# AberHu/TF-NAS

Hardware: AMD Instinct MI355X
Metric: supernet search images/sec (w-step + alpha-step) (higher is better)
Workload: dtype fp32

## Files before the change

tf-nas_amd/csrc/dw_stream.inc:

```

__device__ __forceinline__ int ring_swz(int c) { return c ^ ((c >> 2) & 1); }
struct WinBase {
    const float* b[2][2];
    __device__ __forceinline__ void set(const float* rowp, int d0, int d1) {
        b[0][0] = rowp + d0; b[0][1] = rowp - d0; b[1][0] = rowp + d1; b[1][1] = rowp - d1;
    }
    __device__ __forceinline__ const float* at(int u) const { return b[(u >> 2) & 1][u & 1]; }
};

__device__ __forceinline__ void dws_decode(const DwSlide& gm, int& cy, int& lane) {
    const int L = blockIdx.x;
    if (gm.gx & 7) {
        cy = L % gm.chunks;
        lane = L / gm.chunks;
    } else {
        const int x = L & 7, q = L >> 3;
        cy = q % gm.chunks;
        lane = (q / gm.chunks) * 8 + x;
    }
}

typedef unsigned u32x4 __attribute__((ext_vector_type(4)));
#ifndef TFNAS_LD_AUX
#define TFNAS_LD_AUX 2
// ... 226 lines not shown
                    slot = (slot + 1 == RB) ? 0 : slot + 1;
                }
            } else {
#pragma unroll 1
                for (int ky = 0; ky < K; ++ky) {
                    const float* rowp = ring_item + slot * ge.row_floats;
                    WinBase wb;
                    wb.set(rowp, swz0, swz1);
                    const float* wp = wts_item + ky * K * CC;
                    f32x4 win[K + 3];
#pragma unroll
                    for (int u = 0; u < K + 3; ++u) win[u] = ld4(wb.at(u) + u * CCP);
#pragma unroll
                    for (int kx = 0; kx < K; ++kx) {
                        const f32x4 wv = ld4(wp + kx * CC);
#pragma unroll
                        for (int j = 0; j < 4; ++j) acc[j] += win[j + kx] * wv;
                    }
                    slot = (slot + 1 == RB) ? 0 : slot + 1;
                }
            }
            const unsigned o = ge.row_off(ii, hh) + ooff;
#pragma unroll
            for (int j = 0; j < 4; ++j) {
                if (j < npx) {
                    bD.st4(o + (unsigned)(j * M), acc[j]);
                    ssum += acc[j];
                    ssq += acc[j] * acc[j];
                }
            }
        }
        spos.advance(TH, H, PAD, RB);
        __syncthreads();
        if (PIPE) {
            if (more) {
                rb.commit(ring, ge, bpos, xf);
                bpos.advance(TH, H, PAD, RB);
            }
            __syncthreads();
        }
    }
    dw_flush_stats(ssum, ssq, ring, CC, c0, mcp, off, M, part, lane);
}

template <int K, int ACT, bool PIPE, int KQ = 0, bool WGR = false>
__global__ __launch_bounds__(256, WGR ? 2 : ((PIPE || KQ > 0) ? 3 : 4)) void k_dws_bwd(TfnasCellDesc d, const float* __restrict__ dZ,
                                                    const float* __restrict__ gate, const float* __restrict__ dpooled,
                                                    const float* __restrict__ D, const double* __restrict__ stats2,
                                                    const double* __restrict__ red2, const float* __restrict__ E,
                                                    const double* __restrict__ stats1, float* __restrict__ dEh,
                                                    float* __restrict__ part, DwSlide gm,
                                                    const float* __restrict__ x = nullptr,
                                                    float* __restrict__ wpart = nullptr, size_t wout_size = 0) {
    static_assert(!(PIPE && KQ > 0), "the E-free variant has no register-prefetch form");
    static_assert(!(WGR && KQ > 0), "the fused weight gradient needs a materialised E");
    extern __shared__ __attribute__((aligned(16))) float lds[];
    int cy, lane, g, c0;
    dws_decode(gm, cy, lane);
    if (!dw_locate<K>(d, cy, gm.CC, g, c0)) return;
    const int mc = d.g[g].mc, mcp = d.g[g].mcp, off = d.g[g].off;
    constexpr int CC = 32, CCP = 32, CQ = CC >> 2;
    const int TH = gm.TH, L1 = gm.L1, RB = gm.RB;
    const int H = d.H, W = d.W, M = d.M;
    constexpr int PAD = K / 2;
    const int tid = threadIdx.x;

    float* ring = lds;
    float* wts = lds + RB * L1 * CCP;
    f32x4* cst2 = reinterpret_cast<f32x4*>(wts + K * K * CC);
    float2* cst1 = reinterpret_cast<float2*>(cst2 + CC);
    float* eht = reinterpret_cast<float*>(cst1 + CC);
    fill_cst2(cst2, d, CC, c0, mc, off, stats2, red2);
    if (tid < CC)
        cst1[tid] = (c0 + tid < mc) ? bn_consts(stats1 + 2 * (size_t)(off + c0 + tid), 1.0 / ((double)d.N * H * W), d.eps)
                                    : make_float2(0.f, 0.f);
    for (int idx = tid; idx < K * K * CC; idx += 256) {
        const int cl = idx % CC, t = idx / CC;
        wts[t * CC + cl] = (c0 + cl < mc) ? d.g[g].w_dw[(size_t)(c0 + cl) * (K * K) + (K * K - 1 - t)] : 0.f;
    }
    __syncthreads();
    ExpandB<(KQ > 0 ? KQ : 2)> xb;
    if (KQ > 0) expand_b_load(xb, d.g[g].w_expand, d.ic, c0, mc, cst1);

    StreamGeo ge;
    ge.H = H; ge.PAD = PAD; ge.RB = RB; ge.TH = TH;
    ge.nimg = (d.N - lane + gm.gx - 1) / gm.gx;
    ge.WM = (unsigned)W * M;
    ge.img_stride = (unsigned)gm.gx * H * ge.WM;
    ge.lane_base = (unsigned)lane * H * ge.WM + off + c0;
    ge.row_floats = L1 * CCP;
    const int nsteps = (ge.nimg * (H + PAD) + PAD + TH - 1) / TH;

    const int cq = tid & (CQ - 1);
    const bool has_se = d.g[g].se > 0;
    const float inv_hw = 1.f / (float)(H * W);
    f32x4 c2r[4];
    float2 c1r[4];
#pragma unroll
    for (int j = 0; j < 4; ++j) {
        c2r[j] = cst2[4 * cq + j];
        c1r[j] = cst1[4 * cq + j];
    }
    const float* gate_c = gate + off + c0 + 4 * cq;
    const float* dpool_c = dpooled + off + c0 + 4 * cq;
    auto xf = [&](f32x4 dz, f32x4 dv, int i) {
        f32x4 g4 = zero4(), dp4 = zero4();
        if (has_se) {
            const size_t n = (size_t)(lane + i * gm.gx) * M;
            g4 = ld4(gate_c + n);
            dp4 = ld4(dpool_c + n) * splat4(inv_hw);
        }
        return bn2_dd<ACT>(c2r, 0, dz, dv, has_se, g4, dp4);
    };
    const size_t numel = (size_t)d.N * H * W * M;
    BufView bZ, bDd, bE, bO;
    bZ.bind(dZ, numel);
    bDd.bind(D, numel);
    bE.bind(E, numel);
    bO.bind(dEh, numel);
    RingBlock<true> rb;
    rb.init(gm, W, M, mcp - c0, PAD);
    StreamPos bpos = {0, -PAD, 0};
    if (PIPE) {
        rb.issue(ge, bpos, bZ, bDd);
        rb.commit(ring, ge, bpos, xf);
        bpos.advance(TH, H, PAD, RB);
        __syncthreads();
    }

    const int nsw = gm.TW >> 2, st = tid >> gm.cq_shift;
    const int oh = st / nsw, ow0 = (st - oh * nsw) * 4;
    const bool item_ok = oh < TH && c0 + 4 * cq < mcp;
    const int npx = W - ow0 < 4 ? W - ow0 : 4;
    const float* ring_item = ring + ow0 * CCP + 4 * cq;
    const int swz0 = ((ow0 >> 2) & 1) * CCP, swz1 = CCP - swz0;
    const float* wts_item = wts + 4 * cq;
    const unsigned ooff = (unsigned)(ow0 * M + 4 * cq);
    StreamPos spos = {-1, H - PAD, RB - 2 * PAD};

    f32x4 t1 = zero4(), t2 = zero4();
    f32x4 wacc[WGR ? K * K : 1];
#pragma unroll
    for (int u = 0; u < (WGR ? K * K : 1); ++u) wacc[u] = zero4();
    for (int s = 0; s < nsteps; ++s) {
        const bool more = s + 1 < nsteps;
        if (PIPE) {
            if (more) rb.issue(ge, bpos, bZ, bDd);
        } else {
            rb.issue(ge, bpos, bZ, bDd);
            if (KQ > 0) {
                const int TW = gm.TW;
                const float inv_tw = 1.f / (float)TW;
                expand_tile_to<(KQ > 0 ? KQ : 2), 2>(
                    TH * TW, x, xb,
                    [&](int p, size_t& a) {
                        const int r = (int)(((float)p + 0.5f) * inv_tw), col = p - r * TW;
                        int bi, bh;
                        ge.locate(spos, r, bi, bh);
                        a = (((size_t)(lane + bi * gm.gx) * H + bh) * W + col) * d.ic;
                        return col < W && bh >= 0 && bi >= 0 && bi < ge.nimg;
                    },
                    [&](int p) { return eht + p * CCP; });
            }
            rb.commit(ring, ge, bpos, xf);
            bpos.advance(TH, H, PAD, RB);
            __syncthreads();
        }
        int ii, hh;
        ge.locate(spos, oh, ii, hh);
        if (item_ok && hh >= 0 && ii >= 0 && ii < ge.nimg) {
            const unsigned o = ge.row_off(ii, hh) + ooff;
            f32x4 ev[4];
#pragma unroll
            for (int j = 0; j < 4; ++j) {
                if (KQ > 0) ev[j] = ld4(eht + (oh * gm.TW + ow0 + j) * CCP + 4 * cq);
                else ev[j] = bE.ld4(j < npx ? o + (unsigned)(j * M) : BUF_OOB);
            }
            int slot = ge.slot_of(spos, oh);
            f32x4 acc[4] = {zero4(), zero4(), zero4(), zero4()};
            if (!WGR) {
#pragma unroll 1
                for (int ky = 0; ky < K; ++ky) {
                    const float* rowp = ring_item + slot * ge.row_floats;
                    WinBase wb;
                    wb.set(rowp, swz0, swz1);
                    const float* wp = wts_item + ky * K * CC;
                    f32x4 win[K + 3];
#pragma unroll
                    for (int u = 0; u < K + 3; ++u) win[u] = ld4(wb.at(u) + u * CCP);
#pragma unroll
                    for (int kx = 0; kx < K; ++kx) {
                        const f32x4 wv = ld4(wp + kx * CC);
#pragma unroll
                        for (int j = 0; j < 4; ++j) acc[j] += win[j + kx] * wv;
                    }
                    slot = (slot + 1 == RB) ? 0 : slot + 1;
                }
            } else {
                f32x4 a1v[4];
#pragma unroll
                for (int j = 0; j < 4; ++j)
#pragma unroll
                    for (int q = 0; q < 4; ++q)
                        a1v[j][q] = j < npx ? act_f<ACT>((ev[j][q] - c1r[q].x) * c1r[q].y) : 0.f;
#pragma unroll
                for (int ky = 0; ky < K; ++ky) {
                    const float* rowp = ring_item + slot * ge.row_floats;
                    WinBase wb;
                    wb.set(rowp, swz0, swz1);
                    const float* wp = wts_item + ky * K * CC;
                    f32x4 win[K + 3];
#pragma unroll
                    for (int u = 0; u < K + 3; ++u) win[u] = ld4(wb.at(u) + u * CCP);
#pragma unroll
                    for (int kx = 0; kx < K; ++kx) {
                        const f32x4 wv = ld4(wp + kx * CC);
#pragma unroll
                        for (int j = 0; j < 4; ++j) {
                            acc[j] += win[j + kx] * wv;
                            wacc[(K - 1 - ky) * K + (K - 1 - kx)] += a1v[j] * win[j + kx];
                        }
                    }
                    slot = (slot + 1 == RB) ? 0 : slot + 1;
                    __builtin_amdgcn_sched_barrier(0);
                }
            }
#pragma unroll
            for (int j = 0; j < 4; ++j) {
                if (j < npx) {
                    f32x4 deh;
#pragma unroll
                    for (int q = 0; q < 4; ++q) {
                        const float eh = KQ > 0 ? ev[j][q] : (ev[j][q] - c1r[q].x) * c1r[q].y;
                        deh[q] = acc[j][q] * act_d<ACT>(eh);
                        t1[q] += deh[q];
                        t2[q] += deh[q] * eh;
                    }
                    bO.st4(o + (unsigned)(j * M), deh);
                }
            }
        }
        spos.advance(TH, H, PAD, RB);
        __syncthreads();
        if (PIPE) {
            if (more) {
                rb.commit(ring, ge, bpos, xf);
                bpos.advance(TH, H, PAD, RB);
            }
            __syncthreads();
        }
    }
    dw_flush_stats(t1, t2, ring, CC, c0, mcp, off, M, part, lane);
    if (WGR) {
        for (int o = CQ; o < 64; o <<= 1) {
#pragma unroll
            for (int u = 0; u < K * K; ++u) {
#pragma unroll
                for (int q = 0; q < 4; ++q) wacc[u][q] += __shfl_xor(wacc[u][q], o, 64);
            }
        }
        __syncthreads();
        float* wred = ring;
        const int wl = tid & 63, wv = tid >> 6;
        if (wl < CQ) {
#pragma unroll
            for (int u = 0; u < K * K; ++u) st4(wred + (wv * K * K + u) * CC + 4 * wl, wacc[u]);
        }
        __syncthreads();
        size_t poff = 0;
        for (int gg = 0; gg < g; ++gg) poff += (size_t)d.g[gg].mc * d.g[gg].k * d.g[gg].k;
        float* __restrict__ gw = wpart + (size_t)lane * wout_size + poff;
        for (int idx = tid; idx < K * K * CC; idx += 256) {
            const int cl = idx % CC, u = idx / CC;
            if (c0 + cl < mc) {
                float sum = 0.f;
#pragma unroll
                for (int ww = 0; ww < 4; ++ww) sum += wred[(ww * K * K + u) * CC + cl];
                gw[(size_t)(c0 + cl) * (K * K) + u] = sum;
            }
        }
    }
}

template <int K, int ACT, bool PIPE>
__global__ __launch_bounds__(256, (!PIPE && K == 3) ? 4 : 2) void k_dws_wgrad(TfnasCellDesc d, const float* __restrict__ dZ,
                                                      const float* __restrict__ gate, const float* __restrict__ dpooled,
// ... 161 lines not shown
```

tf-nas_amd/csrc/dwconv_kernels.hip:

```cpp
#include <cstring>
#include <type_traits>
#include "tfnas_dev.h"
#include "kernels.h"
#include "prof.h"
#include "efree.h"

__device__ __forceinline__ int floordiv(int a, int b) { return a >= 0 ? a / b : -((-a + b - 1) / b); }

__device__ __forceinline__ int xcd_first_tile() {
    const int gx = gridDim.x, bx = blockIdx.x;
    return (gx & 7) ? bx : (bx & 7) * (gx >> 3) + (bx >> 3);
}

template <int K>
__device__ __forceinline__ bool dw_locate(const TfnasCellDesc& d, int cy, int CC, int& g, int& c0) {
    for (g = 0; g < d.G; ++g) {
        if (d.g[g].k != K) continue;
        const int t = (d.g[g].mcp + CC - 1) / CC;
        if (cy < t) {
            c0 = cy * CC;
            return true;
        }
        cy -= t;
    }
// ... 664 lines not shown
        else occ = dwd_bwd_occ(kk, d.stride, jw);
        const int want = 1024 * occ * wscale / 100;
        int ns = want / (gms[i].chunks * ncg);
        if (ns > steps / minper) ns = steps / minper;
        ns &= ~3;
        if (ns < 4) ns = 4;
        if (ns < nseg) nseg = ns;
    }
    size_t cap = TFNAS_PART_FLOATS / (row_floats ? row_floats : 1);
    if (cap > 1024) cap = 1024;
    while (nseg > 4 && (size_t)ncg * (nseg >> 2) > cap) nseg -= 4;
    if ((size_t)ncg * (nseg >> 2) > cap) return false;
    for (int i = 0; i < 2; ++i) {
        gms[i].ncg = ncg;
        gms[i].nseg = nseg;
        gms[i].steps = steps_k[i];
        gms[i].per = cdiv(steps_k[i], nseg);
        gms[i].nwg = gms[i].chunks * ncg * (nseg >> 2);
        p.chunks[i] = gms[i].chunks;
    }
    p.fam = DW_DIRECT;
    p.rows = ncg * (nseg >> 2);
    p.jw = jw;
    return true;
}

static DwPlan dw_plan_fwd(const TfnasCellDesc& d, bool efree, bool has_x) {
    DwPlan p = {};
    const size_t row = 2 * (size_t)d.M;
    if (!efree && dwd_fwd_use(d) && dwd_plan(d, row, dwd_jw(d), 1, p)) return p;
    p.kq = efree ? d.ic / 4 : 0;
    if ((!efree || (dws_efree_ic(d.ic) && has_x)) && dws_plan(d, row, p)) {
        p.pipe = !efree && dws_pipe(d);
        return p;
    }
    dw_tile_plan(d, d.Ho, d.Wo, true, 4096, row, efree, p);
    return p;
}

DwPlan dw_plan_bwd_data(const TfnasCellDesc& d, bool efree, bool has_x) {
    DwPlan p = {};
    const size_t row = 2 * (size_t)d.M, wout = dw_wout_size(d);
    const bool direct = !efree && dwd_bwd_use(d);
    if (direct) {
        const int jw = d.stride == 2 ? 2 : dwd_jw(d);
        p.fuse_wgrad = d.need_wgrad && !(d.route & TFNAS_ROUTE_DWWG2_OFF) && d.stride == 2 && dw_groups_k(d, true) &&
                       dwd_plan(d, row + wout + 64, jw, 2, p);
        if (p.fuse_wgrad || dwd_plan(d, row, jw, 2, p)) return p;
    }
    p.kq = efree ? d.ic / 4 : 0;
    if ((!efree || (dws_efree_ic(d.ic) && has_x)) && dws_plan(d, row, p)) {
        p.fuse_wgrad = !direct && !efree && d.need_wgrad && !(d.route & TFNAS_ROUTE_DWWG_OFF) && dw_groups_k(d, false) &&
                       d.W >= 28 && (size_t)p.rows * (row + 64 + wout) <= TFNAS_PART_FLOATS;
        p.pipe = !efree && !p.fuse_wgrad && dws_pipe(d);
        return p;
    }
    dw_tile_plan(d, d.H, d.W, false, 4096, row, efree, p);
    return p;
}

static DwPlan dw_plan_wgrad(const TfnasCellDesc& d) {
    DwPlan p = {};
    const size_t wout = dw_wout_size(d);
    if (dwd_wgrad_use(d) && dwd_plan(d, wout, dwd_jw(d), 0, p)) return p;
    if (dws_plan(d, wout, p)) {
        p.pipe = dws_pipe(d);
        return p;
    }
    dw_tile_plan(d, d.Ho, d.Wo, true, 2048, wout, false, p);
    return p;
}

template <int... Vs, class F>
static bool dw_dispatch(int k, int stride, int act, int v, F&& f) {
    bool hit = false;
    auto with_v = [&](auto K, auto S, auto A) {
        ((v == Vs ? (f(K, S, A, std::integral_constant<int, Vs>{}), hit = true) : false) || ...);
    };
    auto with_a = [&](auto K, auto S) {
        if (act == TFNAS_ACT_RELU) with_v(K, S, std::integral_constant<int, 0>{});
        else with_v(K, S, std::integral_constant<int, 1>{});
    };
    auto with_s = [&](auto K) {
        if (stride == 1) with_a(K, std::integral_constant<int, 1>{});
        else with_a(K, std::integral_constant<int, 2>{});
    };
    if (k == 3) with_s(std::integral_constant<int, 3>{});
    else with_s(std::integral_constant<int, 5>{});
    return hit;
}
constexpr int DW_WG = -1;
static int dws_variant(const DwPlan& p) { return p.fuse_wgrad ? DW_WG : p.kq ? p.kq : (int)p.pipe; }

static int dw_reduce_wgrad(const TfnasCellDesc& d, const float* wpart, int rows, size_t wout, hipStream_t s) {
    size_t poff = 0;
    for (int g = 0; g < d.G; ++g) {
        const int n = d.g[g].mc * d.g[g].k * d.g[g].k;
        const int rc = launch_reduce_rows(wpart + poff, rows, n, wout, nullptr, d.g[g].g_dw, s, wgrad_accum(d));
        if (rc) return rc;
        poff += n;
    }
    return 0;
}

int launch_dw_fwd(const TfnasCellDesc& d, const float* E, const float* x, const double* stats1, float* D,
                  double* stats2, float* part, hipStream_t s) {
    if (!E && !efree_ic_ok(d.ic)) return TFNAS_EINVAL;
    const DwPlan p = dw_plan_fwd(d, E == nullptr, x != nullptr);
    for (int i = 0; i < 2; ++i) {
        if (!p.chunks[i]) continue;
        const int kk = 3 + 2 * i;
        ProfScope _prof(TK_DW_FWD, s, d.G > 2);
        bool ok = false;
        if (p.fam == DW_DIRECT) {
            const DwDirect gm = p.direct[i];
            ok = dw_dispatch<2, 4>(kk, d.stride, d.act, p.jw, [&](auto K, auto S, auto A, auto JW) {
                hipLaunchKernelGGL((k_dwd_fwd<K, S, A, JW>), dim3(gm.nwg), dim3(256), 0, s, d, E, stats1, D, part, gm);
            });
        } else if (p.fam == DW_RING) {
            const DwSlide gm = p.ring[i];
            const size_t shm = (size_t)(gm.RB * gm.L1 * gm.CCP + kk * kk * gm.CC + 2 * gm.CC) * sizeof(float);
            ok = dw_dispatch<0, 1, 6, 10>(kk, d.stride, d.act, dws_variant(p), [&](auto K, auto, auto A, auto V) {
                hipLaunchKernelGGL((k_dws_fwd<K, A, V == 1, V == 1 ? 0 : V>), dim3(p.rows * gm.chunks), dim3(256), shm, s, d, E,
                                   stats1, D, part, gm, V > 1 ? x : nullptr);
            });
        } else {
            const DwGeom gm = p.tile[i];
            const int tile = gm.L0 * gm.L1 * gm.CC > 2048 ? gm.L0 * gm.L1 * gm.CC : 2048;
            const size_t shm = (size_t)(tile + kk * kk * gm.CC + 2 * gm.CC) * sizeof(float);
            if (shm > 64 * 1024) return TFNAS_ERANGE;
            ok = dw_dispatch<0, 4, 6, 10>(kk, d.stride, d.act, p.kq, [&](auto K, auto S, auto A, auto KQ) {
                hipLaunchKernelGGL((k_dw_fwd<K, S, A, KQ>), dim3(p.rows, p.chunks[i]), dim3(256), shm, s, d, E, x, stats1, D,
                                   part, gm);
            });
        }
        if (!ok) return TFNAS_EINVAL;
    }
    return launch_reduce_rows(part, p.rows, 2 * d.M, 2 * (size_t)d.M, stats2, nullptr, s);
}

int launch_dw_bwd_data(const DwPlan& p, const TfnasCellDesc& d, const float* dZ, const float* gate, const float* dpooled,
                       const float* D, const double* stats2, const double* red2, const float* E, const float* x,
                       const double* stats1, float* dEh, double* red1, float* part, hipStream_t s, float* cb1) {
    if (!E && !efree_ic_ok(d.ic)) return TFNAS_EINVAL;
    const size_t wout = dw_wout_size(d);
    float* wpart = part + (((size_t)p.rows * 2 * d.M + 63) & ~(size_t)63);
    for (int i = 0; i < 2; ++i) {
        if (!p.chunks[i]) continue;
        const int kk = 3 + 2 * i;
        ProfScope _prof(TK_DW_BWD_DATA, s, d.G > 2);
        bool ok = false;
        if (p.fam == DW_DIRECT) {
            const DwDirect gm = p.direct[i];
            ok = dw_dispatch<2, 4, DW_WG>(kk, d.stride, d.act, p.fuse_wgrad ? DW_WG : p.jw, [&](auto K, auto S, auto A, auto V) {
                if constexpr (V == DW_WG)
                    hipLaunchKernelGGL((k_dwd_bwd<K, 2, A, 2, true>), dim3(gm.nwg), dim3(256), 0, s, d, dZ, gate, dpooled, D,
                                       stats2, red2, E, stats1, dEh, part, gm, wpart, wout);
                else
                    hipLaunchKernelGGL((k_dwd_bwd<K, S, A, V>), dim3(gm.nwg), dim3(256), 0, s, d, dZ, gate, dpooled, D, stats2,
                                       red2, E, stats1, dEh, part, gm);
            });
        } else if (p.fam == DW_RING) {
            const DwSlide gm = p.ring[i];
            size_t shm = (size_t)(gm.RB * gm.L1 * gm.CCP + kk * kk * gm.CC + 4 * gm.CC + 2 * gm.CC +
                                  (p.kq ? gm.TH * gm.TW * gm.CCP : 0)) * sizeof(float);
            if (p.fuse_wgrad && shm < (size_t)4 * kk * kk * gm.CC * sizeof(float)) shm = (size_t)4 * kk * kk * gm.CC * sizeof(float);
            ok = dw_dispatch<0, 1, 6, 10, DW_WG>(kk, d.stride, d.act, dws_variant(p), [&](auto K, auto, auto A, auto V) {
                if constexpr (V == DW_WG) {
                    if constexpr (K == 3)
                        hipLaunchKernelGGL((k_dws_bwd<K, A, false, 0, true>), dim3(p.rows * gm.chunks), dim3(256), shm, s, d, dZ,
                                           gate, dpooled, D, stats2, red2, E, stats1, dEh, part, gm, nullptr, wpart, wout);
                } else {
                    hipLaunchKernelGGL((k_dws_bwd<K, A, V == 1, V == 1 ? 0 : V>), dim3(p.rows * gm.chunks), dim3(256), shm, s, d,
                                       dZ, gate, dpooled, D, stats2, red2, E, stats1, dEh, part, gm, V > 1 ? x : nullptr);
                }
            });
        } else {
            const DwGeom gm = p.tile[i];
            const int tile = gm.L0 * gm.L1 * gm.CC > 2048 ? gm.L0 * gm.L1 * gm.CC : 2048;
            const size_t shm = (size_t)(tile + kk * kk * gm.CC + 4 * gm.CC + 2 * gm.CC + (p.kq ? gm.T0 * gm.T1 * gm.CC : 0)) *
                               sizeof(float);
            if (shm > 64 * 1024) return TFNAS_ERANGE;
            ok = dw_dispatch<0, 4, 6, 10>(kk, d.stride, d.act, p.kq, [&](auto K, auto S, auto A, auto KQ) {
                hipLaunchKernelGGL((k_dw_bwd_data<K, S, A, KQ>), dim3(p.rows, p.chunks[i]), dim3(256), shm, s, d, dZ, gate,
                                   dpooled, D, stats2, red2, E, x, stats1, dEh, part, gm);
            });
        }
        if (!ok) return TFNAS_EINVAL;
    }
    if (p.fuse_wgrad) {
        ProfScope _prof(TK_DW_WGRAD, s);
        const int rc = dw_reduce_wgrad(d, wpart, p.rows, wout, s);
        if (rc) return rc;
    }
    if (cb1) return launch_reduce_bn1(d, part, p.rows, stats1, red1, cb1, s);
    return launch_reduce_rows(part, p.rows, 2 * d.M, 2 * (size_t)d.M, red1, nullptr, s);
}

int launch_dw_wgrad(const TfnasCellDesc& d, const float* dZ, const float* gate, const float* dpooled, const float* D,
                    const double* stats2, const double* red2, const float* E, const double* stats1, float* part,
                    hipStream_t s) {
    const DwPlan p = dw_plan_wgrad(d);
    const size_t wout = dw_wout_size(d);
    for (int i = 0; i < 2; ++i) {
        if (!p.chunks[i]) continue;
        const int kk = 3 + 2 * i;
        ProfScope _prof(TK_DW_WGRAD, s);
        if (p.fam == DW_DIRECT) {
            const DwDirect gm = p.direct[i];
            dw_dispatch<2, 4>(kk, d.stride, d.act, p.jw, [&](auto K, auto S, auto A, auto JW) {
                hipLaunchKernelGGL((k_dwd_wgrad<K, S, A, JW>), dim3(gm.nwg), dim3(256), 0, s, d, dZ, gate, dpooled, D, stats2,
                                   red2, E, stats1, part, wout, gm);
            });
        } else if (p.fam == DW_RING) {
            const DwSlide gm = p.ring[i];
            int ring = gm.RB * gm.L1 * gm.CCP;
            if (ring < 4 * kk * kk * gm.CC) ring = 4 * kk * kk * gm.CC;
            const size_t shm = (size_t)(ring + 4 * gm.CC + 2 * gm.CC) * sizeof(float);
            dw_dispatch<0, 1>(kk, d.stride, d.act, p.pipe, [&](auto K, auto, auto A, auto PIPE) {
                hipLaunchKernelGGL((k_dws_wgrad<K, A, PIPE == 1>), dim3(p.rows * gm.chunks), dim3(256), shm, s, d, dZ, gate,
                                   dpooled, D, stats2, red2, E, stats1, part, wout, gm);
            });
        } else {
            const DwGeom gm = p.tile[i];
            int tile = gm.L0 * gm.L1 * gm.CC;
            if (tile < 4 * kk * kk * gm.CC) tile = 4 * kk * kk * gm.CC;
            const size_t shm = (size_t)(tile + 4 * gm.CC + 2 * gm.CC) * sizeof(float);
// ... 10 lines not shown
```

tf-nas_amd/csrc/efree.h:

```cpp
#pragma once
#include "tfnas_dev.h"

template <int KQ>
struct ExpandB {
    float b[2][KQ];
    float2 bc[2];
};

template <int KQ>
__device__ __forceinline__ void expand_b_load(ExpandB<KQ>& B, const float* __restrict__ w_expand, int ic, int c0, int mc,
                                              const float2* cst) {
    const int lane = threadIdx.x & 63, n = lane & 15, q = lane >> 4;
#pragma unroll
    for (int nt = 0; nt < 2; ++nt) {
        const int ch = c0 + 16 * nt + n;
#pragma unroll
        for (int kk = 0; kk < KQ; kk += 2) {
            float2 v = make_float2(0.f, 0.f);
            if (ch < mc) v = *reinterpret_cast<const float2*>(w_expand + (size_t)ch * ic + q * KQ + kk);
            B.b[nt][kk] = v.x;
            B.b[nt][kk + 1] = v.y;
        }
        B.bc[nt] = cst[16 * nt + n];
    }
}

template <int KQ, int OUT, class FLoc, class FDst>
__device__ __forceinline__ void expand_tile_to(int npix, const float* __restrict__ x, const ExpandB<KQ>& B, FLoc locate,
                                               FDst dst);
template <int KQ, int OUT, class FLoc>
__device__ __forceinline__ void expand_tile(float* tile, int npix, int CS, const float* __restrict__ x,
                                            const ExpandB<KQ>& B, FLoc locate) {
    expand_tile_to<KQ, OUT>(npix, x, B, locate, [&](int pix) { return tile + pix * CS; });
}
template <int KQ, int OUT, class FLoc, class FDst>
__device__ __forceinline__ void expand_tile_to(int npix, const float* __restrict__ x, const ExpandB<KQ>& B, FLoc locate,
                                               FDst dst) {
    constexpr int NB = KQ <= 4 ? 4 : (KQ <= 6 ? 3 : 2);
    const int lane = threadIdx.x & 63, wave = threadIdx.x >> 6, n = lane & 15, q = lane >> 4;
    const int nmt = (npix + 15) >> 4;
    for (int mt0 = wave; mt0 < nmt; mt0 += 4 * NB) {
        float a[NB][KQ];
        unsigned valid[NB];
#pragma unroll
        for (int b = 0; b < NB; ++b) {
            const int mt = mt0 + 4 * b;
            const int p = 16 * mt + n;
            size_t off = 0;
            const bool ok = mt < nmt && p < npix && locate(p, off);
#pragma unroll
            for (int kk = 0; kk < KQ; kk += 2) {
                float2 v = make_float2(0.f, 0.f);
                if (ok) v = *reinterpret_cast<const float2*>(x + off + q * KQ + kk);
                a[b][kk] = v.x;
                a[b][kk + 1] = v.y;
            }
            valid[b] = (unsigned)(__ballot(ok) & 0xffffull);
        }
#pragma unroll
        for (int b = 0; b < NB; ++b) {
            const int mt = mt0 + 4 * b;
            if (mt >= nmt) break;
            f32x4 acc0 = zero4(), acc1 = zero4();
#pragma unroll
            for (int kk = 0; kk < KQ; ++kk) {
                acc0 = __builtin_amdgcn_mfma_f32_16x16x4f32(a[b][kk], B.b[0][kk], acc0, 0, 0, 0);
                acc1 = __builtin_amdgcn_mfma_f32_16x16x4f32(a[b][kk], B.b[1][kk], acc1, 0, 0, 0);
            }
#pragma unroll
            for (int r = 0; r < 4; ++r) {
                const int pl = 4 * q + r, pix = 16 * mt + pl;
                if (pix < npix) {
                    float v0 = 0.f, v1 = 0.f;
                    if ((valid[b] >> pl) & 1u) {
                        v0 = (acc0[r] - B.bc[0].x) * B.bc[0].y;
                        v1 = (acc1[r] - B.bc[1].x) * B.bc[1].y;
                        if (OUT != 2) {
                            v0 = act_f<(OUT == 2 ? 0 : OUT)>(v0);
                            v1 = act_f<(OUT == 2 ? 0 : OUT)>(v1);
                        }
                    }
                    float* o = dst(pix);
                    o[n] = v0;
                    o[16 + n] = v1;
                }
            }
        }
    }
}

__device__ __forceinline__ void efree_lane_chunk(int& lane, int& cy) {
    const int gx = gridDim.x, chunks = gridDim.y, total = gx * chunks;
    const int L = blockIdx.x + gx * blockIdx.y;
    const int xcd = L & 7, rem = total & 7;
    const int V = xcd * (total >> 3) + (xcd < rem ? xcd : rem) + (L >> 3);
    lane = V / chunks;
    cy = V - lane * chunks;
}
```

tf-nas_amd/tfnas_amd/functions.py:

```python
import ctypes as C
import os

import torch

from . import _lib
from ._lib import TfnasCellDesc, TfnasCellWs, ptr, ptr_array, check

BN_EPS = 1e-5
_EFREE_ENV = os.environ.get('TFNAS_EFREE', '1')
EFREE = _EFREE_ENV != '0'
EFREE_STRIDE1 = _EFREE_ENV == 'all'


def route_from_env(env=None):
    env = os.environ if env is None else env
    r = 0
    for var, bit in (('TFNAS_FX', _lib.ROUTE_FX_OFF), ('TFNAS_FOLD', _lib.ROUTE_FOLD_OFF), ('TFNAS_DWWG', _lib.ROUTE_DWWG_OFF),
                     ('TFNAS_DWWG2', _lib.ROUTE_DWWG2_OFF), ('TFNAS_WGRAD_STREAM', _lib.ROUTE_WGRAD_INLINE)):
        if env.get(var, '1')[:1] == '0':
            r |= bit
    xg = env.get('TFNAS_XG', 'auto')
    r |= _lib.ROUTE_XG_OFF if xg[:1] == '0' else (_lib.ROUTE_XG_ALL if xg == 'all' else 0)
    r |= _lib.ROUTE_DW.get(env.get('TFNAS_DW', 'auto'), 0) | _lib.ROUTE_SE.get(env.get('TFNAS_SE', 'wave'), 0)
    if env.get('TFNAS_GRAM', '1') == '2':
        r |= _lib.ROUTE_GRAM2
    return r


def route_bits(fx=True, fold=True, dwwg=True, dwwg2=True, xg='auto', dw='auto', se='wave', wgrad_stream=True, gram=1):
    return route_from_env({'TFNAS_FX': '1' if fx else '0', 'TFNAS_FOLD': '1' if fold else '0', 'TFNAS_DWWG': '1' if dwwg else '0',
                           'TFNAS_DWWG2': '1' if dwwg2 else '0', 'TFNAS_XG': xg, 'TFNAS_DW': dw, 'TFNAS_SE': se,
                           'TFNAS_WGRAD_STREAM': '1' if wgrad_stream else '0', 'TFNAS_GRAM': str(gram)})


ENV_ROUTE = route_from_env()


def _stream(dev):
    return C.c_void_p(torch.cuda.current_stream(dev).cuda_stream)


class _Null:
    def __enter__(self):
        return None

    def __exit__(self, *a):
        return False


_NULL = _Null()


def _on(dev):
    return _NULL if torch.cuda.current_device() == dev.index else torch.cuda.device(dev)


def _same_device(dev, tensors, what):
    for t in tensors:
        if t is not None and t.device != dev:
            raise RuntimeError('tfnas_amd: %s lives on %s but the input is on %s -- all operands of a launch must share '
                               'one device (one process per GPU; nn.DataParallel replicas must own their parameters)'
                               % (what, t.device, dev))


# ... 73 lines not shown
            ps.extend(b.hip_params())
        return ps

    @property
    def modes(self):
        m = self._modes if self._modes is not None else getattr(self.blocks[0], 'hip_modes', None)
        return m if m is not None else DEFAULT_MODES

    def desc(self, N, H, W):
        key = (N, H, W)
        hit = self._desc_cache.get(key)
        if hit is None:
            d = TfnasCellDesc()
            d.N, d.H, d.W, d.ic, d.oc, d.stride = N, H, W, self.ic, self.oc, self.stride
            d.mode = self.mode
            if self.mode == _lib.MODE_STEM:
                d.Hi, d.Wi = H, W
            d.act, d.has_res, d.G, d.need_wgrad, d.eps = _lib.ACT[self.act], self.has_res, len(self.blocks), 0, BN_EPS
            for g, b in enumerate(self.blocks):
                d.g[g].mc, d.g[g].k, d.g[g].se = b.mid_channels, b.kernel_size, b.se_channels
            self.modes.apply(d)
            check(_lib.lib().tfnas_cell_plan(C.byref(d)), 'tfnas_cell_plan')
            ws = TfnasCellWs()
            check(_lib.lib().tfnas_cell_ws(C.byref(d), C.byref(ws)), 'tfnas_cell_ws')
            hit = (d, ws)
            self._desc_cache[key] = hit
        self.modes.apply(hit[0])
        return hit

    def bind(self, d, params, grads=None):
        i = 0
        for g, b in enumerate(self.blocks):
            n = 1 if self.mode == _lib.MODE_HEAD else (7 if b.se_channels > 0 else 3)
            for j, f in enumerate(_lib._W_FIELDS[:n]):
                setattr(d.g[g], f, params[i + j].data_ptr())
            if grads is not None:
                for j, f in enumerate(_lib._G_FIELDS[:n]):
                    setattr(d.g[g], f, grads[i + j].data_ptr())
            i += n
        d.need_wgrad = int(grads is not None)


def _cell_forward(ctx, plan, xh, N, H, W, wmix, params):
    d, ws = plan.desc(N, H, W)
    for p in params:
        _require_cuda(p, 'MBConv weight')
        if not p.is_contiguous():
            raise RuntimeError('tfnas_amd: MBConv weights must be contiguous')
    plan.bind(d, params)
    d.need_wgrad = int(any(ctx.needs_input_grad[3:]))
    ctx.fwd_route = int(_lib.lib().tfnas_cell_route(C.byref(d)))
    dev = xh.device
    _same_device(dev, list(params) + [wmix], 'a MixedOP weight / mix weight')
    efree = (EFREE and ((plan.stride == 2 and plan.ic <= 24) or EFREE_STRIDE1) and not any(ctx.needs_input_grad[3:])
             and bool(_lib.lib().tfnas_efree_supported(C.byref(d))))
    E = None if efree else torch.empty(ws.E, device=dev, dtype=torch.float32)
    D = torch.empty(ws.D, device=dev, dtype=torch.float32)
    Pr = torch.empty(ws.Pr, device=dev, dtype=torch.float32)
    fsmall = torch.empty(ws.fsmall, device=dev, dtype=torch.float32)
    stats = torch.empty(ws.stats, device=dev, dtype=torch.float64)
    part = _part(ws.part, dev)
    out = torch.empty((N, d.Ho, d.Wo, plan.oc), device=dev, dtype=torch.float32)
    if wmix is not None:
        wmix = wmix.contiguous()
    with _on(dev):
        check(_lib.lib().tfnas_mixedop_fwd(C.byref(d), ptr(xh), ptr(wmix), ptr(E), ptr(D), ptr(Pr), ptr(fsmall),
                                           ptr(stats), ptr(part), ptr(out), _stream(dev)), 'tfnas_mixedop_fwd')
    d.need_wgrad = 0
    ctx.plan, ctx.shape, ctx.has_w = plan, (N, H, W), wmix is not None
    if MixedOpFn.fwd_sink is not None:
        MixedOpFn.fwd_sink.append(dict(plan=plan, d=d, ws=ws, E=E, D=D, stats=stats, fsmall=fsmall, shape=(N, d.H, d.W)))
    ctx.save_for_backward(xh, wmix, E, D, Pr, fsmall, stats, *params)
    return out.permute(0, 3, 1, 2)


def _cell_backward(ctx, dout, want_dx):
    xh, wmix, E, D, Pr, fsmall, stats, *params = ctx.saved_tensors
    plan = ctx.plan
    N, H, W = ctx.shape
    d, ws = plan.desc(N, H, W)
    dev = xh.device
    need_w = any(ctx.needs_input_grad[3:])
    direct = plan.grad_targets if need_w else None
    if direct is not None and (len(direct) != len(params) or any(g.shape != p.shape or g.device != p.device or not g.is_contiguous()
                                                                 for g, p in zip(direct, params))):
        raise RuntimeError('tfnas_amd: grad_targets do not match the parameters of this launch')
    grads = (list(direct) if direct is not None else [torch.empty_like(p) for p in params]) if need_w else None
    plan.bind(d, params, grads)
    douth = _nhwc(dout)
    light = not want_dx and not need_w
    dZ = torch.empty(4 if light else ws.dZ, device=dev, dtype=torch.float32)
    dEh = torch.empty(4 if light else ws.dEh, device=dev, dtype=torch.float32)
    bsmall = torch.empty(ws.bsmall, device=dev, dtype=torch.float32)
    red = torch.empty(ws.red, device=dev, dtype=torch.float64)
    ws_streams = plan.wgrad_streams if need_w else None
    part = _part(ws.part * (4 if ws_streams else (2 if need_w else 1)), dev)
    dx = torch.empty((N, d.H, d.W, plan.ic), device=dev, dtype=torch.float32) if want_dx else None
    dxp = torch.empty(ws.dxp, device=dev, dtype=torch.float32) if want_dx else None
    dwmix = torch.empty(d.G, device=dev, dtype=torch.float32) if ctx.has_w else None
    _same_device(dev, [douth], 'the output gradient')
    d.fwd_route = getattr(ctx, 'fwd_route', 0)
    for k in range(3):
        d.wgrad_stream[k] = ws_streams[k].cuda_stream if (ws_streams and ws_streams[k] is not None) else None
    try:
        with _on(dev):
            check(_lib.lib().tfnas_mixedop_bwd(C.byref(d), ptr(xh), ptr(wmix), ptr(E), ptr(D), ptr(Pr), ptr(fsmall),
                                               ptr(stats), ptr(douth), ptr(dZ), ptr(dEh), ptr(bsmall), ptr(red),
# ... 385 lines not shown
```

tf-nas_amd/tfnas_amd/path.py:

```python
import ctypes as C

import torch

from . import _lib
from ._lib import TfnasCellDesc, TfnasPathDesc, TfnasPathWs, check, ptr, raw_array
from .functions import BN_EPS, DEFAULT_MODES, EFREE, EFREE_STRIDE1, _nhwc, _on, _require_cuda

ALIGN = 64


def _is_arch(name):
    return name.endswith('log_alphas') or name.endswith('betas')


class WeightArena:

    def __init__(self, model):
        named = [(k, p) for k, p in model.named_parameters() if not _is_arch(k)]
        if not named:
            raise ValueError('model has no weight parameters')
        dev = named[0][1].device
        self.device = dev
        self.names, self.params, self.slot = [], [], {}
        off = 0
        for k, p in named:
            _require_cuda(p, 'weight parameter %s' % k)
            n = p.numel()
            self.slot[id(p)] = (off, n)
            self.names.append(k)
            self.params.append(p)
            off += (n + ALIGN - 1) // ALIGN * ALIGN
        self.total = off
        self.w = torch.zeros(off, device=dev, dtype=torch.float32)
        self.g = torch.zeros(off, device=dev, dtype=torch.float32)
        self.m = torch.zeros(off, device=dev, dtype=torch.float32)
        self._gview = {}
        with torch.no_grad():
            for p in self.params:
                o, n = self.slot[id(p)]
                v = self.w[o:o + n].view(p.shape)
                v.copy_(p.data)
                p.data = v
                self._gview[id(p)] = self.g[o:o + n].view(p.shape)
        self._base = self.w.data_ptr()

    def owns(self, p):
        s = self.slot.get(id(p))
        return s is not None and p.data_ptr() == self._base + 4 * s[0]

    def intact(self):
        return all(self.owns(p) for p in self.params)

    def grad_view(self, p):
        return self._gview[id(p)]

    def grad_ptr(self, p):
        return self.g.data_ptr() + 4 * self.slot[id(p)][0]

    def span(self, params):
# ... 62 lines not shown
        cell = self.cells[ci]
        key = (ci, idx, N, H, W)
        blocks = list(cell.m_ops) if idx is None else [cell.m_ops[idx]]
        t = self._tmpl.get(key)
        if t is not None and t.g[0].w_expand == blocks[0].inverted_bottleneck.conv.weight.data_ptr():
            getattr(cell, 'hip_modes', DEFAULT_MODES).apply(t)
            return t
        d = TfnasCellDesc()
        d.N, d.H, d.W, d.ic, d.oc, d.stride = N, H, W, cell.in_channels, cell.out_channels, cell.stride
        d.mode = _lib.MODE_CELL
        d.act, d.G, d.need_wgrad, d.eps = _lib.ACT[cell.act_func], len(blocks), 0, BN_EPS
        d.has_res = int(cell.in_channels == cell.out_channels and cell.stride == 1)
        for g, b in enumerate(blocks):
            d.g[g].mc, d.g[g].k, d.g[g].se = b.mid_channels, b.kernel_size, b.se_channels
            ps = b.hip_params()
            for p in ps:
                _require_cuda(p, 'MBConv weight')
                if not p.is_contiguous():
                    raise RuntimeError('tfnas_amd: MBConv weights must be contiguous')
            for j, f in enumerate(_lib._W_FIELDS[:len(ps)]):
                setattr(d.g[g], f, ps[j].data_ptr())
            if self.weights is not None and all(self.weights.owns(p) for p in ps):
                for j, f in enumerate(_lib._G_FIELDS[:len(ps)]):
                    setattr(d.g[g], f, self.weights.grad_ptr(ps[j]))
        getattr(cell, 'hip_modes', DEFAULT_MODES).apply(d)
        check(self.lib.tfnas_cell_plan(C.byref(d)), 'tfnas_cell_plan')
        self._tmpl[key] = d
        return d

    def _slot(self, name):
        s = self._slots.get(name)
        if s is None:
            s = self._slots[name] = _Slot(self.lib)
        ws = self.wgrad_streams.get(name)
        if ws is not None and getattr(s, 'side', None) is not ws:
            check(self.lib.tfnas_path_set_side_stream(s.ctx, C.c_void_p(ws.cuda_stream)), 'tfnas_path_set_side_stream')
            s.side = ws
        return s

    def _plan(self, name, idxs, x0h, need_wgrad, need_dx0, need_dbetas):
        s = self._slot(name)
        N, H, W, _ = x0h.shape
        soft = idxs is None
        pd = s.pd
        pd.ncell, pd.nstage, pd.soft, pd.need_dx0 = len(self.cells), len(self.stages), int(soft), int(need_dx0)
        mask = 0
        h, w = H, W
        for i, cell in enumerate(self.cells):
            t = self._template(i, None if soft else idxs[i], N, h, w)
            if need_wgrad and not t.g[0].g_expand:
                raise RuntimeError('tfnas_amd: weight gradients at the path level need a WeightArena that owns the weights')
            pd.cell[i] = t
            pd.cell[i].need_wgrad = int(need_wgrad)
            if soft and not need_wgrad and EFREE and ((cell.stride == 2 and cell.in_channels <= 24) or EFREE_STRIDE1) \
                    and self.lib.tfnas_efree_supported(C.byref(t)):
                mask |= 1 << i
            h, w = (h - 1) // cell.stride + 1, (w - 1) // cell.stride + 1
        pd.efree_mask_lo = mask
        if s.dbetas is None:
            s.dbetas = torch.zeros(self.nres_total, device=self.device, dtype=torch.float32)
        off = 0
        for k, st in enumerate(self.stages):
            sg = pd.stage[k]
            sg.ncell, sg.start_res = st.nblocks, st.start_res
            _require_cuda(st.betas, 'betas')
            sg.betas = st.betas.data_ptr()
            sg.dbetas = (s.dbetas.data_ptr() + 4 * off) if need_dbetas else None
            off += st.num_res
        check(self.lib.tfnas_path_plan(s.ctx, C.byref(pd), C.byref(s.ws)), 'tfnas_path_plan')
        if s.arena is None or s.arena.numel() < s.ws.total:
            need = int(s.ws.total)
            if not soft:
                def widest(c):
                    return max(range(len(c.m_ops)), key=lambda i: (c.m_ops[i].mid_channels, c.m_ops[i].se_channels))
                wide = [widest(c) for c in self.cells]
                if list(idxs) != wide:
                    need = max(need, self._sampled_need(name, wide, x0h, need_wgrad, need_dx0))
                    return self._plan_with_arena(name, idxs, x0h, need_wgrad, need_dx0, need_dbetas, need)
            self._grow(s, need)
        s.gen += 1
        return s

    def _grow(self, s, need):
        if s.arena is not None and s.arena.numel() >= need:
            return
        if s.arena is not None:
            torch.cuda.synchronize(self.device)
        s.arena = None
        s.arena = torch.zeros(int(need * 1.02) + 1024, device=self.device, dtype=torch.float32)

    def _sampled_need(self, name, wide, x0h, need_wgrad, need_dx0):
        tmp = '_size_probe'
        s = self._slot(tmp)
        s.arena = torch.empty(0, device=self.device)
        N, H, W, _ = x0h.shape
        pd = s.pd
        pd.ncell, pd.nstage, pd.soft, pd.need_dx0, pd.efree_mask_lo = len(self.cells), len(self.stages), 0, int(need_dx0), 0
        h, w = H, W
        for i, cell in enumerate(self.cells):
            pd.cell[i] = self._template(i, wide[i], N, h, w)
            pd.cell[i].need_wgrad = int(need_wgrad)
            h, w = (h - 1) // cell.stride + 1, (w - 1) // cell.stride + 1
        for k, st in enumerate(self.stages):
            sg = pd.stage[k]
            sg.ncell, sg.start_res, sg.betas, sg.dbetas = st.nblocks, st.start_res, st.betas.data_ptr(), None
        check(self.lib.tfnas_path_plan(s.ctx, C.byref(pd), C.byref(s.ws)), 'tfnas_path_plan')
        return int(s.ws.total)
# ... 196 lines not shown
```

Measured before the change: 3873.

## Recompute expanded activations per item with MFMA in depthwise backward ring kernel

The E-free depthwise backward kernel no longer expands a whole tile into a shared-memory buffer. Each thread now loads its own x slice and recomputes the expanded activation with MFMA chains, then reshuffles the results across lanes with DPP. The E-free variants can also use the pipelined (register-prefetch) ring form, with new dispatch variants for it. This drops the TH*TW shared-memory staging and a barrier-heavy expand phase, which frees LDS and may allow more occupancy. In exchange it adds redundant MFMA work and DPP shuffles on every step. It also adds an efree_policy helper without changing which cells use the E-free path.

```diff
diff --git a/tf-nas_amd/csrc/dw_stream.inc b/tf-nas_amd/csrc/dw_stream.inc
--- a/tf-nas_amd/csrc/dw_stream.inc
+++ b/tf-nas_amd/csrc/dw_stream.inc
@@ -302,7 +302,6 @@
                                                     float* __restrict__ part, DwSlide gm,
                                                     const float* __restrict__ x = nullptr,
                                                     float* __restrict__ wpart = nullptr, size_t wout_size = 0) {
-    static_assert(!(PIPE && KQ > 0), "the E-free variant has no register-prefetch form");
     static_assert(!(WGR && KQ > 0), "the fused weight gradient needs a materialised E");
     extern __shared__ __attribute__((aligned(16))) float lds[];
     int cy, lane, g, c0;
@@ -319,7 +318,6 @@
     float* wts = lds + RB * L1 * CCP;
     f32x4* cst2 = reinterpret_cast<f32x4*>(wts + K * K * CC);
     float2* cst1 = reinterpret_cast<float2*>(cst2 + CC);
-    float* eht = reinterpret_cast<float*>(cst1 + CC);
     fill_cst2(cst2, d, CC, c0, mc, off, stats2, red2);
     if (tid < CC)
         cst1[tid] = (c0 + tid < mc) ? bn_consts(stats1 + 2 * (size_t)(off + c0 + tid), 1.0 / ((double)d.N * H * W), d.eps)
@@ -329,8 +327,22 @@
         wts[t * CC + cl] = (c0 + cl < mc) ? d.g[g].w_dw[(size_t)(c0 + cl) * (K * K) + (K * K - 1 - t)] : 0.f;
     }
     __syncthreads();
-    ExpandB<(KQ > 0 ? KQ : 2)> xb;
-    if (KQ > 0) expand_b_load(xb, d.g[g].w_expand, d.ic, c0, mc, cst1);
+    f32x4* xbl = reinterpret_cast<f32x4*>(cst1 + CC);
+    if constexpr (KQ > 0) {
+        if (tid < 64) {
+            ExpandItemB<(KQ > 0 ? KQ : 2)> xb;
+            expand_item_b_load(xb, d.g[g].w_expand, d.ic, c0, mc);
+            const float* bf = &xb.b[0][0];
+#pragma unroll
+            for (int u = 0; u < KQ / 2; ++u) {
+                f32x4 v;
+#pragma unroll
+                for (int e = 0; e < 4; ++e) v[e] = bf[4 * u + e];
+                xbl[u * 64 + tid] = v;
+            }
+        }
+        __syncthreads();
+    }
 
     StreamGeo ge;
     ge.H = H; ge.PAD = PAD; ge.RB = RB; ge.TH = TH;
@@ -360,7 +372,8 @@
             g4 = ld4(gate_c + n);
             dp4 = ld4(dpool_c + n) * splat4(inv_hw);
         }
-        return bn2_dd<ACT>(c2r, 0, dz, dv, has_se, g4, dp4);
+        if constexpr (KQ > 0 && PIPE) return bn2_dd<ACT>(cst2, 4 * cq, dz, dv, has_se, g4, dp4);
+        else return bn2_dd<ACT>(c2r, 0, dz, dv, has_se, g4, dp4);
     };
     const size_t numel = (size_t)d.N * H * W * M;
     BufView bZ, bDd, bE, bO;
@@ -388,6 +401,27 @@
     const unsigned ooff = (unsigned)(ow0 * M + 4 * cq);
     StreamPos spos = {-1, H - PAD, RB - 2 * PAD};
 
+    ExpandItemA<(KQ > 0 ? KQ : 2)> xa;
+    int xoh[2], xoff[2];
+#pragma unroll
+    for (int t = 0; t < 2; ++t) {
+        const int sa = ((tid >> 6) << 3) + (((tid & 15) >> 2) << 1) + t;
+        const int ow = (sa % nsw) * 4 + (tid & 3);
+        xoh[t] = (sa / nsw < TH && ow < W) ? sa / nsw : -1;
+        xoff[t] = ow * d.ic + ((tid & 63) >> 4) * KQ;
+    }
+    auto x_load = [&](const StreamPos& pos) {
+        const float* px[2];
+#pragma unroll
+        for (int t = 0; t < 2; ++t) {
+            int bi = 0, bh = -1;
+            if (xoh[t] >= 0) ge.locate(pos, xoh[t], bi, bh);
+            const bool ok = bh >= 0 && bi >= 0 && bi < ge.nimg;
+            px[t] = ok ? x + ((size_t)(lane + bi * gm.gx) * H + bh) * W * d.ic + xoff[t] : x;
+        }
+        xa.load(px[0], px[1]);
+    };
+
     f32x4 t1 = zero4(), t2 = zero4();
     f32x4 wacc[WGR ? K * K : 1];
 #pragma unroll
@@ -395,39 +429,27 @@
     for (int s = 0; s < nsteps; ++s) {
         const bool more = s + 1 < nsteps;
         if (PIPE) {
+            if constexpr (KQ > 0) x_load(spos);
             if (more) rb.issue(ge, bpos, bZ, bDd);
         } else {
             rb.issue(ge, bpos, bZ, bDd);
-            if (KQ > 0) {
-                const int TW = gm.TW;
-                const float inv_tw = 1.f / (float)TW;
-                expand_tile_to<(KQ > 0 ? KQ : 2), 2>(
-                    TH * TW, x, xb,
-                    [&](int p, size_t& a) {
-                        const int r = (int)(((float)p + 0.5f) * inv_tw), col = p - r * TW;
-                        int bi, bh;
-                        ge.locate(spos, r, bi, bh);
-                        a = (((size_t)(lane + bi * gm.gx) * H + bh) * W + col) * d.ic;
-                        return col < W && bh >= 0 && bi >= 0 && bi < ge.nimg;
-                    },
-                    [&](int p) { return eht + p * CCP; });
-            }
+            if constexpr (KQ > 0) x_load(spos);
             rb.commit(ring, ge, bpos, xf);
             bpos.advance(TH, H, PAD, RB);
             __syncthreads();
         }
         int ii, hh;
         ge.locate(spos, oh, ii, hh);
-        if (item_ok && hh >= 0 && ii >= 0 && ii < ge.nimg) {
-            const unsigned o = ge.row_off(ii, hh) + ooff;
-            f32x4 ev[4];
-#pragma unroll
-            for (int j = 0; j < 4; ++j) {
-                if (KQ > 0) ev[j] = ld4(eht + (oh * gm.TW + ow0 + j) * CCP + 4 * cq);
-                else ev[j] = bE.ld4(j < npx ? o + (unsigned)(j * M) : BUF_OOB);
+        const bool item_on = item_ok && hh >= 0 && ii >= 0 && ii < ge.nimg;
+        const unsigned o = ge.row_off(ii, hh) + ooff;
+        f32x4 ev[4];
+        f32x4 acc[4] = {zero4(), zero4(), zero4(), zero4()};
+        if (item_on) {
+            if constexpr (KQ == 0) {
+#pragma unroll
+                for (int j = 0; j < 4; ++j) ev[j] = bE.ld4(j < npx ? o + (unsigned)(j * M) : BUF_OOB);
             }
             int slot = ge.slot_of(spos, oh);
-            f32x4 acc[4] = {zero4(), zero4(), zero4(), zero4()};
             if (!WGR) {
 #pragma unroll 1
                 for (int ky = 0; ky < K; ++ky) {
@@ -475,13 +497,28 @@
                     __builtin_amdgcn_sched_barrier(0);
                 }
             }
+        }
+        if constexpr (KQ > 0) {
+            ExpandItemB<(KQ > 0 ? KQ : 2)> xb;
+            float* bf = &xb.b[0][0];
+#pragma unroll
+            for (int u = 0; u < KQ / 2; ++u) {
+                const f32x4 v = xbl[u * 64 + (tid & 63)];
+#pragma unroll
+                for (int e = 0; e < 4; ++e) bf[4 * u + e] = v[e];
+            }
+            f32x4 xt[4];
+            expand_item_chains(xa, xb, xt);
+            expand_item_exchange(xt, ev);
+        }
+        if (item_on) {
 #pragma unroll
             for (int j = 0; j < 4; ++j) {
                 if (j < npx) {
                     f32x4 deh;
 #pragma unroll
                     for (int q = 0; q < 4; ++q) {
-                        const float eh = KQ > 0 ? ev[j][q] : (ev[j][q] - c1r[q].x) * c1r[q].y;
+                        const float eh = (ev[j][q] - c1r[q].x) * c1r[q].y;
                         deh[q] = acc[j][q] * act_d<ACT>(eh);
                         t1[q] += deh[q];
                         t2[q] += deh[q] * eh;
diff --git a/tf-nas_amd/csrc/dwconv_kernels.hip b/tf-nas_amd/csrc/dwconv_kernels.hip
--- a/tf-nas_amd/csrc/dwconv_kernels.hip
+++ b/tf-nas_amd/csrc/dwconv_kernels.hip
@@ -740,7 +740,7 @@
     if ((!efree || (dws_efree_ic(d.ic) && has_x)) && dws_plan(d, row, p)) {
         p.fuse_wgrad = !direct && !efree && d.need_wgrad && !(d.route & TFNAS_ROUTE_DWWG_OFF) && dw_groups_k(d, false) &&
                        d.W >= 28 && (size_t)p.rows * (row + 64 + wout) <= TFNAS_PART_FLOATS;
-        p.pipe = !efree && !p.fuse_wgrad && dws_pipe(d);
+        p.pipe = !p.fuse_wgrad && dws_pipe(d);
         return p;
     }
     dw_tile_plan(d, d.H, d.W, false, 4096, row, efree, p);
@@ -778,7 +778,10 @@
     return hit;
 }
 constexpr int DW_WG = -1;
-static int dws_variant(const DwPlan& p) { return p.fuse_wgrad ? DW_WG : p.kq ? p.kq : (int)p.pipe; }
+constexpr int DWS_KQ_PIPE = 100;
+static int dws_variant(const DwPlan& p) {
+    return p.fuse_wgrad ? DW_WG : p.kq ? p.kq + (p.pipe ? DWS_KQ_PIPE : 0) : (int)p.pipe;
+}
 
 static int dw_reduce_wgrad(const TfnasCellDesc& d, const float* wpart, int rows, size_t wout, hipStream_t s) {
     size_t poff = 0;
@@ -850,17 +853,20 @@
             });
         } else if (p.fam == DW_RING) {
             const DwSlide gm = p.ring[i];
-            size_t shm = (size_t)(gm.RB * gm.L1 * gm.CCP + kk * kk * gm.CC + 4 * gm.CC + 2 * gm.CC +
-                                  (p.kq ? gm.TH * gm.TW * gm.CCP : 0)) * sizeof(float);
+            size_t shm = (size_t)(gm.RB * gm.L1 * gm.CCP + kk * kk * gm.CC + 4 * gm.CC + 2 * gm.CC + 64 * 2 * p.kq) * sizeof(float);
             if (p.fuse_wgrad && shm < (size_t)4 * kk * kk * gm.CC * sizeof(float)) shm = (size_t)4 * kk * kk * gm.CC * sizeof(float);
-            ok = dw_dispatch<0, 1, 6, 10, DW_WG>(kk, d.stride, d.act, dws_variant(p), [&](auto K, auto, auto A, auto V) {
+            ok = dw_dispatch<0, 1, 6, 10, DWS_KQ_PIPE + 6, DWS_KQ_PIPE + 10, DW_WG>(kk, d.stride, d.act, dws_variant(p),
+                                                                                     [&](auto K, auto, auto A, auto V) {
                 if constexpr (V == DW_WG) {
                     if constexpr (K == 3)
                         hipLaunchKernelGGL((k_dws_bwd<K, A, false, 0, true>), dim3(p.rows * gm.chunks), dim3(256), shm, s, d, dZ,
                                            gate, dpooled, D, stats2, red2, E, stats1, dEh, part, gm, nullptr, wpart, wout);
                 } else {
-                    hipLaunchKernelGGL((k_dws_bwd<K, A, V == 1, V == 1 ? 0 : V>), dim3(p.rows * gm.chunks), dim3(256), shm, s, d,
-                                       dZ, gate, dpooled, D, stats2, red2, E, stats1, dEh, part, gm, V > 1 ? x : nullptr);
+                    constexpr int v = decltype(V)::value;
+                    constexpr bool PIPE = v == 1 || v > DWS_KQ_PIPE;
+                    constexpr int KQ = v > DWS_KQ_PIPE ? v - DWS_KQ_PIPE : (v == 1 ? 0 : v);
+                    hipLaunchKernelGGL((k_dws_bwd<K, A, PIPE, KQ>), dim3(p.rows * gm.chunks), dim3(256), shm, s, d, dZ, gate,
+                                       dpooled, D, stats2, red2, E, stats1, dEh, part, gm, KQ ? x : nullptr);
                 }
             });
         } else {
diff --git a/tf-nas_amd/csrc/efree.h b/tf-nas_amd/csrc/efree.h
--- a/tf-nas_amd/csrc/efree.h
+++ b/tf-nas_amd/csrc/efree.h
@@ -23,6 +23,14 @@
         }
         B.bc[nt] = cst[16 * nt + n];
     }
+}
+
+template <int KQ>
+__device__ __forceinline__ f32x4 expand_chain(const float (&a)[KQ], const float (&b)[KQ]) {
+    f32x4 acc = zero4();
+#pragma unroll
+    for (int kk = 0; kk < KQ; ++kk) acc = __builtin_amdgcn_mfma_f32_16x16x4f32(a[kk], b[kk], acc, 0, 0, 0);
+    return acc;
 }
 
 template <int KQ, int OUT, class FLoc, class FDst>
@@ -61,12 +69,7 @@
         for (int b = 0; b < NB; ++b) {
             const int mt = mt0 + 4 * b;
             if (mt >= nmt) break;
-            f32x4 acc0 = zero4(), acc1 = zero4();
-#pragma unroll
-            for (int kk = 0; kk < KQ; ++kk) {
-                acc0 = __builtin_amdgcn_mfma_f32_16x16x4f32(a[b][kk], B.b[0][kk], acc0, 0, 0, 0);
-                acc1 = __builtin_amdgcn_mfma_f32_16x16x4f32(a[b][kk], B.b[1][kk], acc1, 0, 0, 0);
-            }
+            const f32x4 acc0 = expand_chain<KQ>(a[b], B.b[0]), acc1 = expand_chain<KQ>(a[b], B.b[1]);
 #pragma unroll
             for (int r = 0; r < 4; ++r) {
                 const int pl = 4 * q + r, pix = 16 * mt + pl;
@@ -89,6 +92,72 @@
     }
 }
 
+template <int KQ>
+struct ExpandItemB {
+    float b[2][KQ];
+};
+template <int KQ>
+__device__ __forceinline__ void expand_item_b_load(ExpandItemB<KQ>& B, const float* __restrict__ w_expand, int ic, int c0,
+                                                   int mc) {
+    const int lane = threadIdx.x & 63, n = lane & 15, q = lane >> 4;
+#pragma unroll
+    for (int h = 0; h < 2; ++h) {
+        const int ch = c0 + 16 * h + 4 * (n & 3) + (n >> 2);
+#pragma unroll
+        for (int kk = 0; kk < KQ; kk += 2) {
+            float2 v = make_float2(0.f, 0.f);
+            if (ch < mc) v = *reinterpret_cast<const float2*>(w_expand + (size_t)ch * ic + q * KQ + kk);
+            B.b[h][kk] = v.x;
+            B.b[h][kk + 1] = v.y;
+        }
+    }
+}
+template <int KQ>
+struct ExpandItemA {
+    float a[2][KQ];
+    __device__ __forceinline__ void load(const float* p0, const float* p1) {
+#pragma unroll
+        for (int kk = 0; kk < KQ; kk += 2) {
+            const float2 v0 = *reinterpret_cast<const float2*>(p0 + kk), v1 = *reinterpret_cast<const float2*>(p1 + kk);
+            a[0][kk] = v0.x;
+            a[0][kk + 1] = v0.y;
+            a[1][kk] = v1.x;
+            a[1][kk + 1] = v1.y;
+        }
+    }
+};
+template <int CTRL>
+__device__ __forceinline__ float expand_dpp(float v) {
+    return __builtin_bit_cast(float, __builtin_amdgcn_update_dpp(0, __builtin_bit_cast(int, v), CTRL, 0xf, 0xf, true));
+}
+template <bool D8>
+__device__ __forceinline__ void expand_item_stage(f32x4& Ta, f32x4& Tb, bool hi) {
+#pragma unroll
+    for (int r = 0; r < 4; ++r) {
+        const float send = hi ? Ta[r] : Tb[r];
+        const float recv = D8 ? expand_dpp<0x128>(send) : expand_dpp<0x1B>(expand_dpp<0x141>(send));
+        Ta[r] = hi ? recv : Ta[r];
+        Tb[r] = hi ? Tb[r] : recv;
+    }
+}
+template <int KQ>
+__device__ __forceinline__ void expand_item_chains(const ExpandItemA<KQ>& A, const ExpandItemB<KQ>& B, f32x4 (&T)[4]) {
+#pragma unroll
+    for (int m = 0; m < 4; ++m) T[m] = expand_chain<KQ>(A.a[m >> 1], B.b[m & 1]);
+}
+__device__ __forceinline__ void expand_item_exchange(f32x4 (&T)[4], f32x4 (&ev)[4]) {
+    const int n = threadIdx.x & 15;
+    const bool hi8 = n & 8, hi4 = n & 4;
+    expand_item_stage<true>(T[0], T[2], hi8);
+    expand_item_stage<true>(T[1], T[3], hi8);
+    expand_item_stage<false>(T[0], T[1], hi4);
+    expand_item_stage<false>(T[2], T[3], hi4);
+#pragma unroll
+    for (int j = 0; j < 4; ++j)
+#pragma unroll
+        for (int k = 0; k < 4; ++k) ev[j][k] = T[k][j];
+}
+
 __device__ __forceinline__ void efree_lane_chunk(int& lane, int& cy) {
     const int gx = gridDim.x, chunks = gridDim.y, total = gx * chunks;
     const int L = blockIdx.x + gx * blockIdx.y;
diff --git a/tf-nas_amd/tfnas_amd/functions.py b/tf-nas_amd/tfnas_amd/functions.py
--- a/tf-nas_amd/tfnas_amd/functions.py
+++ b/tf-nas_amd/tfnas_amd/functions.py
@@ -10,6 +10,14 @@
 _EFREE_ENV = os.environ.get('TFNAS_EFREE', '1')
 EFREE = _EFREE_ENV != '0'
 EFREE_STRIDE1 = _EFREE_ENV == 'all'
+
+
+def efree_policy(stride, ic, width):
+    if not EFREE:
+        return False
+    if EFREE_STRIDE1:
+        return True
+    return stride == 2 and ic <= 24
 
 
 def route_from_env(env=None):
@@ -189,7 +197,7 @@
     ctx.fwd_route = int(_lib.lib().tfnas_cell_route(C.byref(d)))
     dev = xh.device
     _same_device(dev, list(params) + [wmix], 'a MixedOP weight / mix weight')
-    efree = (EFREE and ((plan.stride == 2 and plan.ic <= 24) or EFREE_STRIDE1) and not any(ctx.needs_input_grad[3:])
+    efree = (efree_policy(plan.stride, plan.ic, W) and not any(ctx.needs_input_grad[3:])
              and bool(_lib.lib().tfnas_efree_supported(C.byref(d))))
     E = None if efree else torch.empty(ws.E, device=dev, dtype=torch.float32)
     D = torch.empty(ws.D, device=dev, dtype=torch.float32)
diff --git a/tf-nas_amd/tfnas_amd/path.py b/tf-nas_amd/tfnas_amd/path.py
--- a/tf-nas_amd/tfnas_amd/path.py
+++ b/tf-nas_amd/tfnas_amd/path.py
@@ -4,7 +4,7 @@
 
 from . import _lib
 from ._lib import TfnasCellDesc, TfnasPathDesc, TfnasPathWs, check, ptr, raw_array
-from .functions import BN_EPS, DEFAULT_MODES, EFREE, EFREE_STRIDE1, _nhwc, _on, _require_cuda
+from .functions import BN_EPS, DEFAULT_MODES, efree_policy, _nhwc, _on, _require_cuda
 
 ALIGN = 64
 
@@ -173,7 +173,7 @@
                 raise RuntimeError('tfnas_amd: weight gradients at the path level need a WeightArena that owns the weights')
             pd.cell[i] = t
             pd.cell[i].need_wgrad = int(need_wgrad)
-            if soft and not need_wgrad and EFREE and ((cell.stride == 2 and cell.in_channels <= 24) or EFREE_STRIDE1) \
+            if soft and not need_wgrad and efree_policy(cell.stride, cell.in_channels, w) \
                     and self.lib.tfnas_efree_supported(C.byref(t)):
                 mask |= 1 << i
             h, w = (h - 1) // cell.stride + 1, (w - 1) // cell.stride + 1
```

After: 3882, median of 2. Within noise of the previous version (+0.2%).
